# mmorise/World

Measured on AMD Instinct MI355X. Metric: analysis frames/sec (Harvest+CheapTrick+D4C, 48 kHz, 5 ms hop), higher is better.
Workload: dtype f64; 1 GPU; configs[1]: 1 x (48 kHz, 10 s) utterance(s) per step, Harvest+CheapTrick+D4C, fft_size=2048, frame_period=5 ms, inputs/outputs in HBM, 12 independent jobs in flight (one HIP stream + context each, a different utterance per job); utterances_per_gpu=1, jobs_in_flight=12, parallelism=single GPU, no collective

## Files before the change

include/world_hip.h:

```cpp
#ifndef WORLD_HIP_H_
#define WORLD_HIP_H_

#ifdef __cplusplus
extern "C" {
#endif

#if defined(__GNUC__)
#define WORLD_HIP_API __attribute__((visibility("default")))
#else
#define WORLD_HIP_API
#endif


typedef struct {
  double f0_floor;
  double f0_ceil;
  double channels_in_octave;
  double frame_period;
  int speed;
  double allowed_range;
} DioOption;

typedef struct {
  double f0_floor;
// ... 183 lines not shown
WORLD_HIP_API int world_hip_cheaptrick_batch(WorldHipContext *ctx, int n_utt, int fs, const double *d_x,
                                             int x_stride, const int *x_length, const int *n_frames,
                                             int f_stride, const double *d_tpos, const double *d_f0,
                                             const CheapTrickOption *option, double *d_spectrogram);
WORLD_HIP_API int world_hip_d4c_batch(WorldHipContext *ctx, int n_utt, int fs, const double *d_x,
                                      int x_stride, const int *x_length, const int *n_frames,
                                      int f_stride, const double *d_tpos, const double *d_f0,
                                      int fft_size, const D4COption *option, double *d_aperiodicity);

WORLD_HIP_API int world_hip_synthesis_batch(WorldHipContext *ctx, int n_utt, int fs, double frame_period,
                                            int fft_size, const int *n_frames, int f_stride, const double *d_f0,
                                            const double *d_spectrogram, const double *d_aperiodicity,
                                            const int *y_length, int y_stride, double *d_y);

WORLD_HIP_API int world_hip_synthesis_records(WorldHipContext *ctx, int n_utt, int fs, double frame_period, int fft_size,
                                              const int *n_frames, long long first_row, const double *d_block, int cols,
                                              int wire, int number_of_dimensions, const int *y_length, int y_stride,
                                              double *d_y);

WORLD_HIP_API int world_hip_probe_machine(WorldHipContext *ctx, double *values, int n_values);
WORLD_HIP_API int world_hip_probe_rfft(WorldHipContext *ctx, int lg_n, int max_lr, int threads, int static_plan,
                                       long long batch, const double *d_in, double *d_spectrum);
WORLD_HIP_API int world_hip_probe_irfft(WorldHipContext *ctx, int lg_n, int max_lr, int threads, int static_plan,
                                        long long batch, const double *d_spectrum, double *d_out);
WORLD_HIP_API int world_hip_probe_fft(WorldHipContext *ctx, int mode, int lg_n, int max_lr, int threads, int swizzle,
                                      long long batch, const void *d_in, void *d_out);
WORLD_HIP_API int world_hip_probe_select(WorldHipContext *ctx, int mode, int threads, int K, long long rows,
                                         const double *d_keys, double *d_out);
WORLD_HIP_API int world_hip_probe_harvest_contour(WorldHipContext *ctx, int n_utt, const int *nfb, const int *nc, int maxc,
                                                  int fb_stride, const double *d_cand, const double *d_score, double frame_period,
                                                  int f_stride, double *d_pruned_cand, double *d_pruned_score, double *d_step2,
                                                  double *d_step3, double *d_step4, int sec_cap, int *d_sec_n, int *d_sec,
                                                  double *d_basic_f0, double *d_tpos, double *d_f0);

WORLD_HIP_API int world_hip_analyze_batch(WorldHipContext *ctx, int n_utt, int fs, const double *d_x, int x_stride,
                                          const int *x_length, const HarvestOption *harvest_option,
                                          const CheapTrickOption *cheaptrick_option, const D4COption *d4c_option,
                                          int f_stride, double *d_tpos, double *d_f0, double *d_spectrogram,
                                          double *d_aperiodicity);
WORLD_HIP_API int world_hip_record_columns(int fft_size, int wire);
WORLD_HIP_API int world_hip_analyze_packed(WorldHipContext *ctx, int n_utt, int fs, const double *d_x, int x_stride,
                                           const int *x_length, const HarvestOption *harvest_option,
                                           const CheapTrickOption *cheaptrick_option, const D4COption *d4c_option,
                                           long long first_row, double *d_block, int cols);
WORLD_HIP_API int world_hip_coded_columns(int fs, int number_of_dimensions);
WORLD_HIP_API int world_hip_analyze_coded(WorldHipContext *ctx, int n_utt, int fs, const double *d_x, int x_stride,
                                          const int *x_length, const HarvestOption *harvest_option,
                                          const CheapTrickOption *cheaptrick_option, const D4COption *d4c_option,
                                          int number_of_dimensions, long long first_row, double *d_block, int cols);
WORLD_HIP_API int world_hip_spectral_packed_range(WorldHipContext *ctx, int n_utt, int fs, const double *d_x, int x_stride,
                                                  const int *x_length, const int *n_frames, int f_stride,
                                                  const double *d_tpos, const double *d_f0,
                                                  const CheapTrickOption *cheaptrick_option, const D4COption *d4c_option,
                                                  int frame_lo, int frame_hi, int reuse_offsets, long long first_row,
                                                  double *d_block, int cols);
WORLD_HIP_API int world_hip_cheaptrick_batch_range(WorldHipContext *ctx, int n_utt, int fs, const double *d_x, int x_stride,
                                                   const int *x_length, const int *n_frames, int f_stride,
                                                   const double *d_tpos, const double *d_f0, const CheapTrickOption *option,
                                                   int frame_lo, int frame_hi, int reuse_offsets, double *d_spectrogram);
WORLD_HIP_API int world_hip_d4c_batch_range(WorldHipContext *ctx, int n_utt, int fs, const double *d_x, int x_stride,
                                            const int *x_length, const int *n_frames, int f_stride, const double *d_tpos,
                                            const double *d_f0, int fft_size, const D4COption *option, int frame_lo,
                                            int frame_hi, int reuse_offsets, double *d_aperiodicity);
WORLD_HIP_API int world_hip_pack_results(WorldHipContext *ctx, int n_utt, const int *n_frames, int f_stride,
                                         int bins, const double *d_tpos, const double *d_f0,
                                         const double *d_spectrogram, const double *d_aperiodicity,
// ... 186 lines not shown
```

world_amd/api.py:

```python
import ctypes as C
import os
import weakref

import numpy as np

HERE = os.path.dirname(os.path.abspath(__file__))
LIB_PATH = os.environ.get("WORLD_HIP_LIB") or os.path.join(HERE, "libworld_hip.so")

_dp = C.POINTER(C.c_double)
_ip = C.POINTER(C.c_int)


class DioOption(C.Structure):
    _fields_ = [("f0_floor", C.c_double), ("f0_ceil", C.c_double), ("channels_in_octave", C.c_double),
                ("frame_period", C.c_double), ("speed", C.c_int), ("allowed_range", C.c_double)]


class HarvestOption(C.Structure):
    _fields_ = [("f0_floor", C.c_double), ("f0_ceil", C.c_double), ("frame_period", C.c_double)]


class CheapTrickOption(C.Structure):
    _fields_ = [("q1", C.c_double), ("f0_floor", C.c_double), ("fft_size", C.c_int)]

# ... 213 lines not shown
    lib.world_hip_create.restype = vp
    lib.world_hip_create.argtypes = [C.c_int, vp]
    lib.world_hip_destroy.argtypes = [vp]
    lib.world_hip_last_error.restype = C.c_char_p
    lib.world_hip_sync.argtypes = [vp]
    lib.world_hip_workspace_bytes.restype = C.c_ulonglong
    lib.world_hip_workspace_bytes.argtypes = [vp]
    lib.world_hip_noise_table_bytes.restype = C.c_ulonglong
    lib.world_hip_noise_table_bytes.argtypes = [vp]
    lib.world_hip_verify_tables.argtypes = [vp]
    lib.world_hip_harvest_batch.argtypes = [vp, C.c_int, C.c_int, vp, C.c_int, _ip, C.POINTER(HarvestOption),
                                            C.c_int, vp, vp]
    lib.world_hip_dio_batch.argtypes = [vp, C.c_int, C.c_int, vp, C.c_int, _ip, C.POINTER(DioOption),
                                        C.c_int, vp, vp]
    lib.world_hip_stonemask_batch.argtypes = [vp, C.c_int, C.c_int, vp, C.c_int, _ip, _ip, C.c_int, vp, vp, vp]
    lib.world_hip_cheaptrick_batch.argtypes = [vp, C.c_int, C.c_int, vp, C.c_int, _ip, _ip, C.c_int, vp, vp,
                                               C.POINTER(CheapTrickOption), vp]
    lib.world_hip_d4c_batch.argtypes = [vp, C.c_int, C.c_int, vp, C.c_int, _ip, _ip, C.c_int, vp, vp, C.c_int,
                                        C.POINTER(D4COption), vp]
    lib.world_hip_synthesis_batch.argtypes = [vp, C.c_int, C.c_int, C.c_double, C.c_int, _ip, C.c_int, vp, vp, vp,
                                              _ip, C.c_int, vp]
    lib.world_hip_pcm16_to_double.argtypes = [vp, C.c_longlong, vp, vp]
    lib.world_hip_set_synthesis_pulse_capacity.argtypes = [vp, C.c_int]
    lib.world_hip_synthesis_pulses_dropped.argtypes = [vp, _ip]
    lib.world_hip_probe_rfft.argtypes = [vp, C.c_int, C.c_int, C.c_int, C.c_int, C.c_longlong, vp, vp]
    lib.world_hip_probe_irfft.argtypes = [vp, C.c_int, C.c_int, C.c_int, C.c_int, C.c_longlong, vp, vp]
    if hasattr(lib, "world_hip_probe_fft"):
        lib.world_hip_probe_fft.argtypes = [vp, C.c_int, C.c_int, C.c_int, C.c_int, C.c_int, C.c_longlong, vp, vp]
    if hasattr(lib, "world_hip_probe_select"):
        lib.world_hip_probe_select.argtypes = [vp, C.c_int, C.c_int, C.c_int, C.c_longlong, vp, vp]
    if hasattr(lib, "world_hip_probe_harvest_contour"):
        lib.world_hip_probe_harvest_contour.argtypes = [vp, C.c_int, _ip, _ip, C.c_int, C.c_int, vp, vp, C.c_double, C.c_int,
                                                        vp, vp, vp, vp, vp, C.c_int, vp, vp, vp, vp, vp]
    lib.world_hip_analyze_packed.argtypes = [vp, C.c_int, C.c_int, vp, C.c_int, _ip, C.POINTER(HarvestOption),
                                             C.POINTER(CheapTrickOption), C.POINTER(D4COption), C.c_longlong, vp, C.c_int]
    lib.world_hip_analyze_sharded.argtypes = [C.c_int, C.POINTER(vp), C.c_int, C.c_int, C.POINTER(vp), _ip,
                                              C.POINTER(HarvestOption), C.POINTER(CheapTrickOption), C.POINTER(D4COption),
                                              C.c_int, C.POINTER(vp), C.c_longlong, C.c_int, C.POINTER(C.c_longlong)]
    lib.world_hip_check_shape.argtypes = [C.c_int, C.c_int, C.c_char_p, C.c_int]
    if hasattr(lib, "world_hip_set_hint"):
        lib.world_hip_set_hint.argtypes = [vp, C.c_int]
    if hasattr(lib, "world_hip_probe_machine"):
        lib.world_hip_probe_machine.argtypes = [vp, C.POINTER(C.c_double), C.c_int]
    lib.world_hip_record_columns.argtypes = [C.c_int, C.c_int]
    if hasattr(lib, "world_hip_analyze_coded"):
        lib.world_hip_coded_columns.argtypes = [C.c_int, C.c_int]
        lib.world_hip_analyze_coded.argtypes = [vp, C.c_int, C.c_int, vp, C.c_int, _ip, C.POINTER(HarvestOption),
                                                C.POINTER(CheapTrickOption), C.POINTER(D4COption), C.c_int, C.c_longlong, vp, C.c_int]
    lib.world_hip_spectral_packed_range.argtypes = [vp, C.c_int, C.c_int, vp, C.c_int, _ip, _ip, C.c_int, vp, vp,
                                                    C.POINTER(CheapTrickOption), C.POINTER(D4COption), C.c_int, C.c_int,
                                                    C.c_int, C.c_longlong, vp, C.c_int]
    lib.world_hip_cheaptrick_batch_range.argtypes = [vp, C.c_int, C.c_int, vp, C.c_int, _ip, _ip, C.c_int, vp, vp,
                                                     C.POINTER(CheapTrickOption), C.c_int, C.c_int, C.c_int, vp]
    lib.world_hip_d4c_batch_range.argtypes = [vp, C.c_int, C.c_int, vp, C.c_int, _ip, _ip, C.c_int, vp, vp, C.c_int,
                                              C.POINTER(D4COption), C.c_int, C.c_int, C.c_int, vp]
    lib.world_hip_analyze_batch.argtypes = [vp, C.c_int, C.c_int, vp, C.c_int, _ip, C.POINTER(HarvestOption),
                                            C.POINTER(CheapTrickOption), C.POINTER(D4COption), C.c_int, vp, vp, vp, vp]
    lib.world_hip_graph_begin.argtypes = [vp]
    lib.world_hip_graph_end.argtypes = [vp, C.POINTER(vp)]
    lib.world_hip_graph_launch.argtypes = [vp, vp]
    lib.world_hip_graph_destroy.argtypes = [vp]
    lib.world_hip_pack_results.argtypes = [vp, C.c_int, _ip, C.c_int, C.c_int, vp, vp, vp, vp, C.c_longlong, vp]
    lib.world_hip_unpack_results.argtypes = [vp, C.c_int, _ip, C.c_int, C.c_int, vp, C.c_longlong, vp, vp, vp, vp]
    lib.world_hip_allgather_blocks.argtypes = [C.c_int, C.POINTER(vp), C.POINTER(vp), C.POINTER(C.c_longlong), C.c_int,
                                               C.POINTER(vp)]
    lib.world_hip_pcm_to_double.argtypes = [vp, C.c_longlong, C.c_int, vp, vp]
# ... 1014 lines not shown
                                                 out.data_ptr()), "probe_fft")
        return out

    def probe_select(self, keys, K, mode=0):
        t = self.torch
        assert keys.dtype == t.float64 and keys.is_contiguous() and keys.dim() == 3 and keys.shape[2] == 10
        out = t.empty((keys.shape[0], 3), dtype=t.float64, device=keys.device)
        self._check(self.lib.world_hip_probe_select(self._context(), mode, keys.shape[1], K, keys.shape[0], keys.data_ptr(),
                                                    out.data_ptr()), "probe_select")
        return out

    def probe_harvest_contour(self, cand, score, nfb, nc, frame_period=5.0):
        t = self.torch
        assert cand.dtype == score.dtype == t.float64 and cand.is_contiguous() and score.is_contiguous()
        assert cand.dim() == 3 and cand.shape == score.shape and len(nfb) == len(nc) == cand.shape[0]
        n, stride, maxc = cand.shape
        nfb, nc = [int(v) for v in nfb], [int(v) for v in nc]
        frames = [int((f - 1) / frame_period) + 1 for f in nfb]
        sec_cap, f_stride = max(nfb) // 2 + 4, max(max(frames), 1)
        nan = lambda *shape: t.full(shape, float("nan"), dtype=t.float64, device=cand.device)
        out = dict(pruned_cand=nan(n, stride, maxc), pruned_score=nan(n, stride, maxc), step2=nan(n, stride), step3=nan(n, stride),
                   step4=nan(n, stride), sec_n=t.full((n, 2), -1, dtype=t.int32, device=cand.device),
                   sec=t.full((n, 6, sec_cap), -1, dtype=t.int32, device=cand.device), basic_f0=nan(n, stride),
                   tpos=nan(n, f_stride), f0=nan(n, f_stride))
        ints = lambda v: (C.c_int * n)(*v)
        self._check(self.lib.world_hip_probe_harvest_contour(
            self._context(), n, ints(nfb), ints(nc), maxc, stride, cand.data_ptr(), score.data_ptr(), frame_period, f_stride,
            out["pruned_cand"].data_ptr(), out["pruned_score"].data_ptr(), out["step2"].data_ptr(), out["step3"].data_ptr(),
            out["step4"].data_ptr(), sec_cap, out["sec_n"].data_ptr(), out["sec"].data_ptr(), out["basic_f0"].data_ptr(),
            out["tpos"].data_ptr(), out["f0"].data_ptr()), "probe_harvest_contour")
        out["n_frames"] = frames
        return out

    def capture(self, fn):
        ctx = self._context()
        self._check(self.lib.world_hip_graph_begin(ctx), "graph_begin")
        g = C.c_void_p()
        try:
            fn()
        except BaseException:
            if self.lib.world_hip_graph_end(ctx, C.byref(g)) == 0 and g:
                self.lib.world_hip_graph_destroy(g)
            raise
        self._check(self.lib.world_hip_graph_end(ctx, C.byref(g)), "graph_end")
        return Graph(self, ctx, g)

    def analyze_packed(self, x, fs, block, first_row=0, x_len=None, frame_period=5.0, f0_floor=71.0, f0_ceil=800.0,
                       q1=-0.15, threshold=0.85, fft_size=None):
        t = self.torch
        B, L, xl = self._prep(x, x_len)
        fft_size = fft_size or cheaptrick_fft_size(fs, 71.0)
        nb = fft_size // 2 + 1
        nf = [frame_count(fs, int(n), frame_period) for n in xl]
        cols = block.shape[-1]
        assert block.dtype == t.float64 and block.is_contiguous() and cols in (2 + 2 * nb, 2 + nb) and block.device == x.device
        assert first_row >= 0 and first_row + sum(nf) <= block.shape[0]
        hopt, copt, dopt = HarvestOption(f0_floor, f0_ceil, frame_period), CheapTrickOption(q1, 71.0, fft_size), D4COption(threshold)
        self._check(self.lib.world_hip_analyze_packed(self._context(), B, fs, x.data_ptr(), L, xl.ctypes.data_as(_ip),
                                                      C.byref(hopt), C.byref(copt), C.byref(dopt), first_row,
                                                      block.data_ptr(), cols), "analyze_packed")
        return nf

    def analyze_coded(self, x, fs, block, first_row=0, x_len=None, frame_period=5.0, f0_floor=71.0, f0_ceil=800.0,
                      q1=-0.15, threshold=0.85, number_of_dimensions=60, fft_size=None):
        t = self.torch
        B, L, xl = self._prep(x, x_len)
# ... 627 lines not shown
```

world_amd/csrc/api.hip:

```cpp
#include "../../include/world_hip.h"

#include <algorithm>
#include <climits>
#include <cmath>
#include <cstdint>
#include <cstring>
#include <cstdarg>
#include <deque>
#include <mutex>
#include <thread>
#include <unordered_map>
#include <stdexcept>
#include <string>
#include <vector>

#include "common.h"
#include "bandfilter.h"
#include "codec.h"
#include "decimate.h"
#include "dio.h"
#include "exchange.h"
#include "fft_probe.h"
#include "d4c_select_probe.h"
#include "gmm_host.h"
// ... 427 lines not shown
  p.park_ws = slot ? a.take<double>(slot * p.park_slots) : nullptr;
}
static void spectral_workspace(WorldHipContext *c, CtParams *ct, D4cParams *d4c, const int *x_length, const int *n_frames) {
  ensure_arena(c, d4c ? measure([&](Arena &a) { carve_d4c(a, *d4c); }) : measure([&](Arena &a) { carve_cheaptrick(a, *ct); }));
  const BatchView &b = ct ? ct->b : d4c->b;
  WorldHipContext::PrepToken t;
  t.n_utt = b.n_utt; t.fs = b.fs; t.f_stride = b.f_stride; t.x_stride = b.x_stride; t.x = b.x;
  t.lengths_hash = lengths_hash(x_length, n_frames, b.n_utt);
  if (ct) {
    c->arena.reset();
    carve_cheaptrick(c->arena, *ct);
    t.fft = 1 << ct->lg_fft; t.f0 = ct->f0; t.tpos = ct->tpos; t.opt = ct->f0_floor;
    t.lo = 0; t.hi = c->arena.used;
    claim_prepared(c, c->prep_ct, c->prep_d4c, t, ct->skip_prepare != 0, "CheapTrick");
    if (!ct->skip_prepare) devrt::dpoison(c->arena.base + c->arena.floor, c->arena.used - c->arena.floor, c->stream);
  }
  if (d4c) {
    c->arena.reset();
    carve_d4c(c->arena, *d4c);
    t.fft = d4c->fft_out; t.f0 = d4c->f0; t.tpos = d4c->tpos; t.opt = d4c->threshold;
    t.lo = reinterpret_cast<char *>(d4c->ap0) - c->arena.base; t.hi = c->arena.used;
    claim_prepared(c, c->prep_d4c, c->prep_ct, t, d4c->skip_prepare != 0, "D4C");
    char *lo = reinterpret_cast<char *>(d4c->skip_prepare ? d4c->coarse : d4c->ap0);
    devrt::dpoison(lo, c->arena.base + c->arena.used - lo, c->stream);
  }
}

static std::string shape_limit(int what, int fs, int fft_size);
static void refuse_shape_limit(int what, int fs, int fft_size) {
  const std::string lim = shape_limit(what, fs, fft_size);
  if (!lim.empty()) fail("%s", lim.c_str());
}
static bool inkernel_consts() { return getenv("WORLD_HIP_INKERNEL_CONSTS") != nullptr; }
static CtParams setup_cheaptrick(WorldHipContext *c, int n_utt, int fs, const double *d_x, int x_stride,
                                 const int *x_length, const int *n_frames, int f_stride, const double *d_tpos,
                                 const double *d_f0, const CheapTrickOption *opt, double *d_sp, const RowLayout &lay,
                                 int *max_frames_out) {
  check_batch(n_utt, fs, d_x, x_stride, x_length);
  const int lg = ilog2_exact(opt->fft_size);
  const std::string lim = shape_limit(2, fs, opt->fft_size);
  if (!lim.empty()) fail("%s", lim.c_str());
  const int max_frames = *max_frames_out = max_frame_count(n_frames, n_utt, f_stride);
  CtParams p;
  p.b = batch_view(c, n_utt, fs, d_x, x_stride, x_length, n_frames, f_stride);
  p.tpos = d_tpos; p.f0 = d_f0; p.spectrogram = d_sp;
  p.out_row = lay.rows ? upload(c, std::vector<int>(lay.rows, lay.rows + n_utt)) : nullptr;
  p.out_stride = lay.stride ? lay.stride : (size_t)(opt->fft_size / 2 + 1);
  p.out_col_bytes = lay.col_bytes; p.out_f32 = lay.f32;
  p.code_ndim = lay.code_dims; p.code_knot = lay.code_knot; p.code_frac = lay.code_frac;
  p.code_w_re = lay.code_w_re; p.code_w_im = lay.code_w_im;
  if (p.code_ndim > 0 && (lay.f32 || !lay.code_knot || p.code_ndim > opt->fft_size / 4 + 1)) fail("CheapTrick: bad coded-row layout");
  p.f0_floor = 3.0 * fs / (opt->fft_size - 3.0);
  p.noise = ensure_noise(c, (size_t)max_frames * ct_max_draws_per_frame(opt->fft_size));
  p.tab = c->tab;
  p.q1 = opt->q1;
  p.lg_fft = lg;
  p.frec = nullptr;
  p.frame_consts = inkernel_consts() ? 0 : 1;
  p.frame_threads = ct_frame_threads(lg);
  p.lift0 = (1.0 - 2.0 * opt->q1) + 2.0 * opt->q1;
  if (lay.frame_lo < 0 || lay.frame_hi < lay.frame_lo) fail("bad frame range [%d, %d)", lay.frame_lo, lay.frame_hi);
  p.frame_lo = lay.frame_lo; p.frame_hi = lay.frame_hi; p.skip_prepare = lay.skip_prepare ? 1 : 0;
  return p;
}
static void run_cheaptrick(WorldHipContext *c, int n_utt, int fs, const double *d_x, int x_stride,
                           const int *x_length, const int *n_frames, int f_stride, const double *d_tpos,
// ... 261 lines not shown
  static const int ev_group_env = [] { const char *e = getenv("WORLD_HIP_EVENT_GROUP"); return e ? std::max(1, atoi(e)) : 40; }();
  p.ev_group = std::min(n_utt, ev_group_env);
  p.ev_u0 = 0;
  const size_t E = p.ev_group;
  p.nyq_slices = (max_y + 4095) / 4096;
  p.mean_parts = p.ratio == 1 ? p.nyq_slices : (max_x + 2 * p.lag + 2 * kDecPad + kDecSpan - 1) / kDecSpan;
  begin_stage(c, [&](Arena &a) {
    p.nyq = a.take<double>(B * p.nyq_slices * 4);
    p.mean_part = a.take<double>(B * p.mean_parts);
    p.quirk = a.take<double>(B * p.nch * kQuirkDoubles);
    p.fwd = a.take<double>(B * p.m_stride);
    p.y = a.take<double>(B * p.y_stride);
    p.events = a.take<double>(E * p.nch * 4 * p.ev_cap);
    p.ev_count = a.take<int>(E * p.nch * 4);
    if (direct_lists) {
      p.seg_events = p.events; p.seg_count = p.ev_count;
    } else {
      p.seg_events = a.take<double>(E * p.nch * 4 * p.nseg * p.seg_cap);
      p.seg_count = a.take<int>(E * p.nch * 4 * p.nseg);
    }
    p.blk_spec = a.take<double2>(B * p.nblk * kBandFftBins);
    p.raw = a.take<double>(B * p.nch * p.fb_stride);
    carve_harvest_tail(a, p, B);
  });
  p.b = batch_view(c, n_utt, fs, d_x, x_stride, x_length, nfr.data(), f_stride);
  p.y_len = upload(c, yl);
  p.nfb = upload(c, nfb);
  p.ref_fft = upload(c, rfft);
  p.band_f0 = hb.d_band_f0; p.band_half = hb.d_half; p.band_off = hb.d_off; p.band_taps = hb.d_taps;
  p.win_tab = hb.d_win_tab; p.win_lane = hb.d_win_tab + (size_t)hb.win_tab_len * 6;
  p.win_full = hb.win_full_entries && !getenv("WORLD_HIP_REFINE_ROTATE")
                   ? reinterpret_cast<const double2 *>(p.win_lane + (size_t)hb.win_tab_len * WAVE * 2) : nullptr;
  p.refine_frames = getenv("WORLD_HIP_REFINE_FRAMES") != nullptr;
  p.inkernel_consts = inkernel_consts() ? 1 : 0;
  p.tpos = d_tpos; p.f0 = d_f0;
  launch_harvest(p, max_x, max_y, max_fb, max_fr, c->stream);
#ifdef WORLD_EMU
  if (const char *dump = getenv("WORLD_EMU_DUMP")) {
    auto put = [&](const char *tag, const void *ptr, size_t bytes) {
      std::string fn = std::string(dump) + "_" + tag + ".bin";
      FILE *f = fopen(fn.c_str(), "wb"); fwrite(ptr, 1, bytes, f); fclose(f);
    };
    int hdr[6] = {p.nch, p.fb_stride, p.maxc, max_fb, p.y_stride, yl[0]};
    put("hdr", hdr, sizeof hdr);
    put("y", p.y, sizeof(double) * p.y_stride);
    put("raw", p.raw, sizeof(double) * p.nch * p.fb_stride);
    put("cand_a", p.cand_a, sizeof(double) * p.fb_stride * p.maxc);
    put("cand_b", p.cand_b, sizeof(double) * p.fb_stride * p.maxc);
    put("score_a", p.score_a, sizeof(double) * p.fb_stride * p.maxc);
    put("score_b", p.score_b, sizeof(double) * p.fb_stride * p.maxc);
    put("basic", p.basic_f0, sizeof(double) * p.fb_stride);
    put("nc", p.nc, sizeof(int));
  }
#endif
}

static void prepare_dio_bands(WorldHipContext *c, int fs, const DioOption *opt, int ratio) {
  DioBands &db = c->dio_bands;
  if (db.fs == fs && db.ratio == ratio && db.f0_floor == opt->f0_floor && db.f0_ceil == opt->f0_ceil &&
      db.cpo == opt->channels_in_octave && db.nb > 0)
    return;
  const double afs = static_cast<double>(fs) / ratio;
  const int nb = 1 + static_cast<int>(log(opt->f0_ceil / opt->f0_floor) / kLog2 * opt->channels_in_octave);
  std::vector<double> fb(nb), taps, lowcut;
  std::vector<int> hal(nb), off(nb);
  int max_ntap = 0;
// ... 1903 lines not shown
    const size_t B = n_utt, row = p.fb_stride, cand_bytes = sizeof(double) * B * row * maxc;
    refuse_overlap(me,
                   {{d_pruned_cand, cand_bytes, "pruned_cand"}, {d_pruned_score, cand_bytes, "pruned_score"},
                    {d_step2, sizeof(double) * B * row, "step2"}, {d_step3, sizeof(double) * B * row, "step3"},
                    {d_step4, sizeof(double) * B * row, "step4"}, {d_basic_f0, sizeof(double) * B * row, "basic_f0"},
                    {d_sec_n, sizeof(int) * B * 2, "sec_n"}, {d_sec, sizeof(int) * B * 6 * p.sec_cap, "sec"},
                    {d_tpos, sizeof(double) * B * f_stride, "tpos"}, {d_f0, sizeof(double) * B * f_stride, "f0"}},
                   {{d_cand, cand_bytes, "cand"}, {d_score, cand_bytes, "score"}});
    begin_stage(c, [&](Arena &a) { carve_harvest_tail(a, p, B); });
    p.b.n_utt = n_utt; p.b.f_stride = f_stride;
    p.b.n_frames = upload(c, nfr);
    p.nfb = upload(c, fb);
    devrt::d2d(p.nc, upload(c, cn), sizeof(int) * B, c->stream);
    for (size_t u = 0; u < B; ++u) {
      const size_t at = u * row * maxc, n = sizeof(double) * fb[u] * maxc;
      devrt::d2d(p.cand_b + at, d_cand + at, n, c->stream);
      devrt::d2d(p.score_b + at, d_score + at, n, c->stream);
    }
    p.tpos = d_tpos; p.f0 = d_f0;
    launch_harvest_tail(p, max_fb, max_fr, c->stream);
    for (size_t u = 0; u < B; ++u) {
      const size_t at = u * row * maxc, n = sizeof(double) * fb[u] * maxc, f = u * row, nf = sizeof(double) * fb[u];
      if (cn[u]) {
        devrt::d2d(d_pruned_cand + at, p.cand_a + at, n, c->stream);
        devrt::d2d(d_pruned_score + at, p.score_a + at, n, c->stream);
      }
      devrt::d2d(d_step2 + f, p.c2 + f, nf, c->stream);
      devrt::d2d(d_step3 + f, p.c3 + f, nf, c->stream);
      devrt::d2d(d_step4 + f, p.c0 + f, nf, c->stream);
      devrt::d2d(d_basic_f0 + f, p.basic_f0 + f, nf, c->stream);
    }
    devrt::d2d(d_sec_n, p.sec_n, sizeof(int) * B * 2, c->stream);
    devrt::d2d(d_sec, p.sec, sizeof(int) * B * 6 * p.sec_cap, c->stream);
  });
}

int world_hip_pack_results(WorldHipContext *c, int n_utt, const int *n_frames, int f_stride, int bins,
                           const double *d_tpos, const double *d_f0, const double *d_spectrogram,
                           const double *d_aperiodicity, long long first_row, double *d_block) {
  return guarded(c, [&] {
    run_pack(c, false, n_utt, n_frames, f_stride, bins, d_tpos, d_f0, d_spectrogram, d_aperiodicity, first_row, d_block);
  });
}

int world_hip_unpack_results(WorldHipContext *c, int n_utt, const int *n_frames, int f_stride, int bins,
                             const double *d_block, long long first_row, double *d_tpos, double *d_f0,
                             double *d_spectrogram, double *d_aperiodicity) {
  return guarded(c, [&] {
    run_pack(c, true, n_utt, n_frames, f_stride, bins, d_tpos, d_f0, d_spectrogram, d_aperiodicity, first_row,
             const_cast<double *>(d_block));
  });
}

int world_hip_allgather_blocks(int n_dev, WorldHipContext *const *ctxs, const double *const *d_src, const long long *rows,
                               int cols, double *const *d_dst) {
  try {
    if (n_dev <= 0 || !ctxs || !d_src || !rows || !d_dst || cols <= 0) fail("bad arguments");
    std::vector<long long> first(n_dev + 1, 0);
    for (int d = 0; d < n_dev; ++d) {
      if (!ctxs[d] || rows[d] < 0 || (rows[d] > 0 && !d_src[d]) || !d_dst[d]) fail("bad block %d", d);
      for (int e = 0; e < d; ++e)
        if (ctxs[e] == ctxs[d]) fail("context %d listed twice", d);
      first[d + 1] = first[d] + rows[d];
    }
    std::vector<std::unique_lock<std::mutex>> locks;
    {
// ... 460 lines not shown
```

world_amd/csrc/bandfilter.h:

```cpp
#pragma once
#include "trace.h"
#include "common.h"

namespace world_hip {

constexpr int kBpThreads = 256;
constexpr int kOutPer = 8;
constexpr int kTile = kBpThreads * kOutPer;
constexpr int kSegTiles = 2;
constexpr int kSeg = kTile * kSegTiles;
constexpr int kSegCap = kSeg / 2 + 2;

__host__ __device__ __forceinline__ int pad8(int i) { return i + (i >> 3); }

struct BandJob {
  const double *in;
  int in_len;
  int n;
  const double *taps;
  int ntap;
  int shift;
  int max_ntap;
  int nseg;
  double *seg_events;
// ... 347 lines not shown
    base = base < lo + 1 ? lo + 1 : base;
    base = base > hi - 32 ? hi - 32 : base;
    const int ones = ones_at(base + sub, true);
    if (ones == 0) hi = base;
    else if (ones == 32) lo = base + 31;
    else return base + ones;
  }
  while (hi - lo > 32) {
    const int stride = (hi - lo + 31) / 32;
    const int idx = lo + (sub + 1) * stride;
    const int ones = ones_at(idx, idx < hi);
    const int nlo = lo + ones * stride, nhi = lo + (ones + 1) * stride;
    lo = nlo;
    hi = nhi < hi ? nhi : hi;
  }
  return lo + 1 + ones_at(lo + 1 + sub, lo + 1 + sub < hi);
#endif
}

__device__ __forceinline__ double interp_intervals(const double *e, int n_int, double fs, double t) {
  const int lo = intervals_at_or_before(e, n_int, fs, t);
  int k = lo < 1 ? 1 : (lo > n_int - 1 ? n_int - 1 : lo);
  double x0 = interval_loc(e, k - 1, fs), x1 = interval_loc(e, k, fs);
  double y0 = interval_f0(e, k - 1, fs), y1 = interval_f0(e, k, fs);
  double sl = (t - x0) / (x1 - x0);
  return y0 + sl * (y1 - y0);
}

struct IntervalRange {
  int c_first, c_last;
  int j_lo, m;
};
#ifndef HV_INTERVAL_CAP
#define HV_INTERVAL_CAP 288
#endif
constexpr int kIntervalCap = HV_INTERVAL_CAP;

__device__ __forceinline__ void interval_range_ends(const double *e, int n_int, double fs, double t, bool last,
                                                    IntervalRange *r) {
  const int c = intervals_at_or_before(e, n_int, fs, t);
  if (last) r->c_last = c; else r->c_first = c;
}
__device__ __forceinline__ void interval_range_close(int n_int, IntervalRange *r) {
  const int k_first = r->c_first < 1 ? 1 : (r->c_first > n_int - 1 ? n_int - 1 : r->c_first);
  const int k_last = r->c_last < 1 ? 1 : (r->c_last > n_int - 1 ? n_int - 1 : r->c_last);
  r->j_lo = k_first - 1;
  r->m = k_last - r->j_lo + 1;
}
__device__ __forceinline__ double interp_staged(const IntervalRange &r, const double *loc, const double *f0,
                                                int n_int, double t) {
  int lo = r.c_first, hi = r.c_last;
  while (lo < hi) {
    const int mid = (lo + hi) >> 1;
    if (loc[mid - r.j_lo] <= t) lo = mid + 1; else hi = mid;
  }
  const int k = (lo < 1 ? 1 : (lo > n_int - 1 ? n_int - 1 : lo)) - r.j_lo;
  const double x0 = loc[k - 1], x1 = loc[k], y0 = f0[k - 1], y1 = f0[k];
  const double sl = (t - x0) / (x1 - x0);
  return y0 + sl * (y1 - y0);
}

}
```

world_amd/csrc/harvest.h:

```cpp
#pragma once
#include "common.h"

namespace world_hip {

constexpr int kQuirkDoubles = 8;
constexpr int kBandFftThreads = 256;
struct HarvestParams {
  BatchView b;
  double f0_floor, f0_ceil, frame_period;
  int ratio;
  double afs;
  int nch;
  int maxc;
  int lag;
  int y_stride;
  int fb_stride;
  int ev_cap;
  int refine_cap;
  int sec_cap;
  int lone_job;
  int ext_cap;
  const int *y_len;
  const int *nfb;
  const double *band_f0;
  const int *band_half;
  const int *band_off;
  const double *band_taps;
  const double2 *band_spec;
  double2 *blk_spec;
  int fft_seg;
  int fft_pre;
  int max_half;
  const int *ref_fft;
  double *nyq;
  int nyq_slices;
  double *mean_part;
  int mean_parts;
  double *quirk;
  int inkernel_consts;
  const double *win_tab;
  const double *win_lane;
  const double2 *win_full;
  int refine_frames;
  Tables tab;
  double *fwd;
  int m_stride;
  double *y;
  double *seg_events;
  int *seg_count;
  int nseg;
  int seg_cap;
  int nblk;
  int chunk_blocks;
  double *events;
  int *ev_count;
  int ev_group;
  int ev_u0;
  double *raw;
  double *cand_a, *score_a;
  double *cand_b, *score_b;
  int *nc;
  double *c0, *c2, *c3;
  int *sec;
  int *sec_n;
  double *sec_sum;
  double *ext;
  double *basic_f0;
  double *tpos;
  double *f0;
};

inline int hv_sliced_sections(int max_fb) { return max_fb / 7 + 4; }
inline int hv_section_rows(int max_fb) { return max_fb / 2 + 4; }
constexpr int kBandFftLg = 12, kBandFft = 1 << kBandFftLg, kBandFftBins = kBandFft / 2 + 1;
int hv_fft_segment(int max_half);
void launch_band_spectra(const double *d_taps, const int *d_off, const int *d_half, int nch, double2 *d_spec,
                         const Tables &tab, hipStream_t stream);
void launch_harvest(const HarvestParams &p, int max_x_len, int max_y_len, int max_fb, int max_frames,
                    hipStream_t stream);
void launch_harvest_tail(const HarvestParams &p, int max_fb, int max_frames, hipStream_t stream);
void launch_harvest_contour(const HarvestParams &p, int max_fb, int max_frames, hipStream_t stream);

}
```

world_amd/csrc/harvest.hip:

```cpp
#ifndef HV_PLAIN_TID
#define WH_FRESH_TID
#endif
#include "bandfilter.h"
#include "decimate.h"
#include "harvest.h"
#include "trace.h"
WH_TRACE_DEFINE(hv)

namespace world_hip {

__global__ void __launch_bounds__(kDecThreads) hv_decimate_fwd(HarvestParams p, IirCoef c) {
  DYN_LDS(lds);
  const int u = blockIdx.y;
  dec_forward_block(p.b.x + (size_t)u * p.b.x_stride, p.b.x_len[u], p.lag, c, blockIdx.x,
                    p.fwd + (size_t)u * p.m_stride, reinterpret_cast<double *>(lds), dec_warm(p.ratio));
}
__global__ void __launch_bounds__(kDecThreads) hv_decimate_bwd(HarvestParams p, IirCoef c) {
  DYN_LDS(lds);
  const int u = blockIdx.y;
  dec_backward_block(p.fwd + (size_t)u * p.m_stride, p.b.x_len[u], p.lag, p.ratio, c, blockIdx.x,
                     p.lag / p.ratio, p.y_len[u], p.y + (size_t)u * p.y_stride, reinterpret_cast<double *>(lds),
                     dec_warm(p.ratio), p.mean_part + (size_t)u * p.mean_parts);
}
__global__ void hv_copy_signal(HarvestParams p) {
// ... 256 lines not shown
#endif
constexpr int kRawRun = HV_RAW_RUN;
__device__ __forceinline__ double hv_gate(const HarvestParams &p, int band, double v0, double v1, double v2, double v3) {
  double c = (v0 + v1 + v2 + v3) / 4.0;
  const double fb = p.band_f0[band];
  if (c > fb * 1.1 || c < fb * 0.9 || c > p.f0_ceil || c < p.f0_floor) c = 0.0;
  return c;
}
#ifndef HV_RAW_MIN_WG
#define HV_RAW_MIN_WG 8
#endif
__global__ void __launch_bounds__(kRawFrames, HV_RAW_MIN_WG) hv_raw_candidates(HarvestParams p) {
  DYN_LDS(lds);
  const int band = blockIdx.x, ue = blockIdx.z, u = ue + p.ev_u0, tid = threadIdx.x, nt = blockDim.x;
  if (band >= p.nch) return;
  const int f_begin = blockIdx.y * kRawRun, f_end = imin(f_begin + kRawRun, p.nfb[u]);
  if (f_begin >= f_end) return;
  const int *cnt = p.ev_count + (ue * p.nch + band) * 4;
  const double *ev = p.events + ((size_t)(ue * p.nch + band) * 4) * p.ev_cap;
  double *out = p.raw + ((size_t)u * p.nch + band) * p.fb_stride;
  int n_int[4];
  bool ok = true;
  for (int fam = 0; fam < 4; ++fam) {
    n_int[fam] = cnt[fam] >= 2 ? cnt[fam] - 1 : 0;
    if (n_int[fam] - 2 <= 0) ok = false;
  }
  if (!ok) {
    for (int f = f_begin + tid; f < f_end; f += nt) out[f] = 0.0;
    return;
  }
  double *loc = reinterpret_cast<double *>(lds);
  double *fz = loc + 4 * kIntervalCap;
  IntervalRange *range = reinterpret_cast<IntervalRange *>(fz + 4 * kIntervalCap);
#ifdef WORLD_EMU
  for (int job = tid; job < 8; job += nt) {
    const int fam = job >> 1;
    const bool last = job & 1;
    interval_range_ends(ev + (size_t)fam * p.ev_cap, n_int[fam], p.afs, (last ? f_end - 1 : f_begin) * 1 / 1000.0, last,
                        range + fam);
  }
#else
  {
    static_assert(kRawFrames == 8 * 32, "one 32-lane group per (family, end)");
    const int job = tid >> 5, fam = job >> 1, sub = tid & 31;
    const bool last = job & 1;
    const int c = intervals_at_or_before_group(ev + (size_t)fam * p.ev_cap, n_int[fam], p.afs,
                                               (last ? f_end - 1 : f_begin) * 1 / 1000.0, (tid >> 5) & 1, sub);
    if (sub == 0) { if (last) range[fam].c_last = c; else range[fam].c_first = c; }
  }
#endif
  __syncthreads();
  for (int fam = tid; fam < 4; fam += nt) interval_range_close(n_int[fam], range + fam);
  __syncthreads();
  const bool staged = range[0].m <= kIntervalCap && range[1].m <= kIntervalCap && range[2].m <= kIntervalCap &&
                      range[3].m <= kIntervalCap;
  if (!staged) {
    for (int f = f_begin + tid; f < f_end; f += nt) {
      const double t = f * 1 / 1000.0;
      out[f] = hv_gate(p, band, interp_intervals(ev, n_int[0], p.afs, t), interp_intervals(ev + p.ev_cap, n_int[1], p.afs, t),
                       interp_intervals(ev + 2 * (size_t)p.ev_cap, n_int[2], p.afs, t),
                       interp_intervals(ev + 3 * (size_t)p.ev_cap, n_int[3], p.afs, t));
    }
    return;
  }
  {
    const int m0 = range[0].m, m1 = m0 + range[1].m, m2 = m1 + range[2].m, m3 = m2 + range[3].m;
    for (int job = tid; job < m3; job += nt) {
      const int fam = (job >= m0) + (job >= m1) + (job >= m2);
      const int i = job - (fam == 0 ? 0 : fam == 1 ? m0 : fam == 2 ? m1 : m2);
      const double *e = ev + (size_t)fam * p.ev_cap + range[fam].j_lo;
      loc[fam * kIntervalCap + i] = interval_loc(e, i, p.afs);
      fz[fam * kIntervalCap + i] = interval_f0(e, i, p.afs);
    }
  }
  __syncthreads();
  for (int f = f_begin + tid; f < f_end; f += nt) {
    const double t = f * 1 / 1000.0;
    double v[4];
#pragma unroll
    for (int fam = 0; fam < 4; ++fam)
      v[fam] = interp_staged(range[fam], loc + fam * kIntervalCap, fz + fam * kIntervalCap, n_int[fam], t);
    out[f] = hv_gate(p, band, v[0], v[1], v[2], v[3]);
  }
}

__global__ void hv_detect(HarvestParams p) {
  const int frame = flat_thread_x(), u = blockIdx.y;
  if (frame >= p.nfb[u]) return;
  const double *raw = p.raw + (size_t)u * p.nch * p.fb_stride + frame;
  double *out = p.cand_a + ((size_t)u * p.fb_stride + frame) * p.maxc;
  int cnt = 0, st = 0, prev = 0;
  double run_sum = 0.0;
  constexpr int kBatch = 19;
  auto fetch = [&](double (&v)[kBatch], int j0) __attribute__((always_inline)) {
#pragma unroll
    for (int q = 0; q < kBatch; ++q) v[q] = raw[(size_t)imin(j0 + q, p.nch - 1) * p.fb_stride];
  };
  auto walk = [&](const double (&v)[kBatch], int j0) __attribute__((always_inline)) {
#pragma unroll
    for (int q = 0; q < kBatch; ++q) {
      const int j = j0 + q;
      if (j >= p.nch || j == 0) continue;
      const int cur = (j == p.nch - 1) ? 0 : (v[q] > 0 ? 1 : 0);
      if (cur - prev == 1) { st = j; run_sum = 0.0; }
      if (cur - prev == -1 && j - st >= 10 && cnt < p.maxc) out[cnt++] = run_sum / (j - st);
      if (cur) run_sum += v[q];
      prev = cur;
    }
  };
  double va[kBatch], vb[kBatch];
  fetch(va, 0);
  for (int j0 = 0; j0 < p.nch; j0 += 2 * kBatch) {
    fetch(vb, j0 + kBatch);
    walk(va, j0);
// ... 510 lines not shown
      }
    }
  }
  __syncthreads();
  {
    const int lane = lane_id(), nfr = imin(kPruneFrames, nfb - f0);
    for (int r = wave_in_block(); r < nfr; r += waves_per_block()) {
      const double *c = rows + (size_t)(r + 1) * nslot, *sv = kept_sc + (size_t)r * nslot;
      double best = 0.0, top = 0.0;
      int slot = 0x7FFFFFFF;
      for (int j = lane; j < nslot; j += WAVE) {
        const double sj = sv[j];
        if (sj > top) { best = c[j]; top = sj; slot = j; }
      }
      const double wtop = wave_max(top);
      double v = 0.0;
      if (wtop > 0.0) {
        const int mine = top == wtop ? slot : 0x7FFFFFFF;
        const int win = -wave_max_int(-mine);
#ifndef WORLD_EMU
        v = readlane_f64(best, __builtin_amdgcn_readfirstlane(win % WAVE));
#else
        (void)win;
        v = best;
#endif
      }
      if (lane == 0) p.c0[(size_t)u * p.fb_stride + f0 + r] = v;
    }
  }
}

size_t hv_band_lds_bytes(int max_half) { return band_lds_bytes(2 * max_half + 1); }

void launch_harvest(const HarvestParams &p, int max_x_len, int max_y_len, int max_fb, int max_frames,
                    hipStream_t stream) {
  const int B = p.b.n_utt;
  if (p.ratio == 1) {
    WH_THREADS(hv_copy_signal, max_y_len, B, 1, stream, p);
  } else {
    IirCoef c = decimate_coef(p.ratio);
    const int spans = (max_x_len + 2 * p.lag + 2 * kDecPad + kDecSpan - 1) / kDecSpan;
    WH_BLOCKS(hv_decimate_fwd, dim3(spans, B), kDecThreads, dec_lds_bytes(), stream, p, c);
    WH_BLOCKS(hv_decimate_bwd, dim3(spans, B), kDecThreads, dec_lds_bytes(), stream, p, c);
  }
  if (p.ratio == 1) WH_BLOCKS(hv_partial_sums, dim3(p.mean_parts, B), 256, 64 * sizeof(double), stream, p);
  WH_BLOCKS(hv_remove_mean, dim3(p.nyq_slices, B), 256, 64 * sizeof(double), stream, p);
  const size_t lds = sizeof(double) * (kBandFft + 64 + twiddle_lds_doubles(kBandFftLg - 1));
  if (p.fft_seg > 0) WH_BLOCKS(hv_block_spectra, dim3(p.nblk + p.nch, B), 256, lds, stream, p);
  else WH_BLOCKS(hv_band_quirk, dim3(p.nch, B), 64, 64 * sizeof(double), stream, p);
  for (int u0 = 0; u0 < B; u0 += p.ev_group) {
    HarvestParams g = p;
    g.ev_u0 = u0;
    const int G = imin(p.ev_group, B - u0);
    if (p.fft_seg > 0 && p.inkernel_consts)
      devrt::launch_blocks("hv_band_events_fft", hv_band_events_fft<false>, dim3(p.nch, p.nseg, G), kBandFftThreads, lds, stream, g);
    else if (p.fft_seg > 0)
      devrt::launch_blocks("hv_band_events_fft", hv_band_events_fft<true>, dim3(p.nch, p.nseg, G), kBandFftThreads, lds, stream, g);
    else WH_BLOCKS(hv_band_events, dim3(p.nseg, p.nch, G), kBpThreads, hv_band_lds_bytes(p.max_half), stream, g);
    if (!(p.fft_seg > 0 && p.nseg == 1)) WH_BLOCKS(hv_compact_events, dim3(p.nch * 4, G), 256, compact_lds_bytes(p.nseg), stream, g);
    WH_BLOCKS(hv_raw_candidates, dim3((p.nch + 7) / 8 * 8, (max_fb + kRawRun - 1) / kRawRun, G), kRawFrames,
              8 * kIntervalCap * sizeof(double) + 4 * sizeof(IntervalRange), stream, g);
  }
  WH_THREADS(hv_detect, max_fb, B, 1, stream, p);
  if (p.win_full && !p.refine_frames)
    WH_WAVES(hv_refine, max_fb, B, 1, sizeof(double) * (3 * p.refine_cap + 6 * static_cast<int>(p.afs / 1000.0) + 2), stream, p);
  else
    WH_WAVES(hv_refine_frames, max_fb, B, 1, 3 * sizeof(double) * p.refine_cap, stream, p);
  launch_harvest_tail(p, max_fb, max_frames, stream);
}

void launch_harvest_tail(const HarvestParams &p, int max_fb, int max_frames, hipStream_t stream) {
  const int B = p.b.n_utt;
  WH_BLOCKS(hv_prune, dim3((max_fb + kPruneFrames - 1) / kPruneFrames, B), 256,
            sizeof(double) * (size_t)(2 * kPruneFrames + 2) * p.maxc, stream, p);
  launch_harvest_contour(p, max_fb, max_frames, stream);
}

}
```

Baseline: 4.441 million frames/s.

## Locate interpolation intervals in Harvest raw candidates by histogram scan instead of bisection

The raw-candidate kernel now histograms, per frame, how many event intervals start before it, using packed 16-bit LDS atomics, then runs a block-wide prefix scan so each frame reads its bracketing interval directly instead of bisecting per family. An optional early gate, enabled by an environment variable, writes zero for frames whose interpolated candidates provably fall outside the band's gate range. The interval cap shrinks slightly to make room for the extra LDS, and a probe entry point is added for testing the routes. The trade is per-block atomics, a scan, and more LDS against the removed binary searches; the counting path is the default.

```diff
diff --git a/include/world_hip.h b/include/world_hip.h
--- a/include/world_hip.h
+++ b/include/world_hip.h
@@ -239,6 +239,9 @@
                                                   int f_stride, double *d_pruned_cand, double *d_pruned_score, double *d_step2,
                                                   double *d_step3, double *d_step4, int sec_cap, int *d_sec_n, int *d_sec,
                                                   double *d_basic_f0, double *d_tpos, double *d_f0);
+WORLD_HIP_API int world_hip_probe_raw_candidates(WorldHipContext *ctx, int route, int n_band, int ev_cap, const double *d_events,
+                                                 const int *ev_count, const double *d_band_f0, int nfb, double afs,
+                                                 double f0_floor, double f0_ceil, int fb_stride, double *d_raw);
 
 WORLD_HIP_API int world_hip_analyze_batch(WorldHipContext *ctx, int n_utt, int fs, const double *d_x, int x_stride,
                                           const int *x_length, const HarvestOption *harvest_option,
diff --git a/world_amd/api.py b/world_amd/api.py
--- a/world_amd/api.py
+++ b/world_amd/api.py
@@ -269,6 +269,9 @@
     if hasattr(lib, "world_hip_probe_harvest_contour"):
         lib.world_hip_probe_harvest_contour.argtypes = [vp, C.c_int, _ip, _ip, C.c_int, C.c_int, vp, vp, C.c_double, C.c_int,
                                                         vp, vp, vp, vp, vp, C.c_int, vp, vp, vp, vp, vp]
+    if hasattr(lib, "world_hip_probe_raw_candidates"):
+        lib.world_hip_probe_raw_candidates.argtypes = [vp, C.c_int, C.c_int, C.c_int, vp, _ip, vp, C.c_int, C.c_double, C.c_double,
+                                                       C.c_double, C.c_int, vp]
     lib.world_hip_analyze_packed.argtypes = [vp, C.c_int, C.c_int, vp, C.c_int, _ip, C.POINTER(HarvestOption),
                                              C.POINTER(CheapTrickOption), C.POINTER(D4COption), C.c_longlong, vp, C.c_int]
     lib.world_hip_analyze_sharded.argtypes = [C.c_int, C.POINTER(vp), C.c_int, C.c_int, C.POINTER(vp), _ip,
@@ -1349,6 +1352,19 @@
         out["n_frames"] = frames
         return out
 
+    def probe_raw_candidates(self, events, counts, band_f0, nfb, afs=8000.0, f0_floor=71.0, f0_ceil=800.0, route=1):
+        t = self.torch
+        assert events.dtype == band_f0.dtype == t.float64 and events.is_contiguous() and band_f0.is_contiguous()
+        assert events.dim() == 3 and events.shape[1] == 4 and band_f0.shape == (events.shape[0],)
+        n, _, ev_cap = events.shape
+        flat = [int(v) for row in counts for v in row]
+        assert len(flat) == 4 * n
+        raw = t.full((n, int(nfb)), float("nan"), dtype=t.float64, device=events.device)
+        self._check(self.lib.world_hip_probe_raw_candidates(
+            self._context(), route, n, ev_cap, events.data_ptr(), (C.c_int * len(flat))(*flat), band_f0.data_ptr(), int(nfb), afs,
+            f0_floor, f0_ceil, int(nfb), raw.data_ptr()), "probe_raw_candidates")
+        return raw
+
     def capture(self, fn):
         ctx = self._context()
         self._check(self.lib.world_hip_graph_begin(ctx), "graph_begin")
diff --git a/world_amd/csrc/api.hip b/world_amd/csrc/api.hip
--- a/world_amd/csrc/api.hip
+++ b/world_amd/csrc/api.hip
@@ -483,6 +483,8 @@
   if (!lim.empty()) fail("%s", lim.c_str());
 }
 static bool inkernel_consts() { return getenv("WORLD_HIP_INKERNEL_CONSTS") != nullptr; }
+static bool raw_bisect() { return getenv("WORLD_HIP_RAW_BISECT") != nullptr; }
+static bool raw_early_gate() { return getenv("WORLD_HIP_RAW_EARLY_GATE") != nullptr; }
 static CtParams setup_cheaptrick(WorldHipContext *c, int n_utt, int fs, const double *d_x, int x_stride,
                                  const int *x_length, const int *n_frames, int f_stride, const double *d_tpos,
                                  const double *d_f0, const CheapTrickOption *opt, double *d_sp, const RowLayout &lay,
@@ -810,6 +812,8 @@
   p.win_full = hb.win_full_entries && !getenv("WORLD_HIP_REFINE_ROTATE")
                    ? reinterpret_cast<const double2 *>(p.win_lane + (size_t)hb.win_tab_len * WAVE * 2) : nullptr;
   p.refine_frames = getenv("WORLD_HIP_REFINE_FRAMES") != nullptr;
+  p.raw_bisect = raw_bisect() ? 1 : 0;
+  p.raw_early_gate = raw_early_gate() ? 1 : 0;
   p.inkernel_consts = inkernel_consts() ? 1 : 0;
   p.tpos = d_tpos; p.f0 = d_f0;
   launch_harvest(p, max_x, max_y, max_fb, max_fr, c->stream);
@@ -2779,6 +2783,41 @@
     }
     devrt::d2d(d_sec_n, p.sec_n, sizeof(int) * B * 2, c->stream);
     devrt::d2d(d_sec, p.sec, sizeof(int) * B * 6 * p.sec_cap, c->stream);
+  });
+}
+
+int world_hip_probe_raw_candidates(WorldHipContext *c, int route, int n_band, int ev_cap, const double *d_events, const int *ev_count,
+                                   const double *d_band_f0, int nfb, double afs, double f0_floor, double f0_ceil, int fb_stride,
+                                   double *d_raw) {
+  return guarded(c, [&] {
+    const char *const me = "probe_raw_candidates";
+    if (route < 0 || route > 3)
+      fail("%s: route = %d unsupported (0: as the environment says, 1: counted, 2: bisected, 3: counted with the early gate)", me, route);
+    if (n_band < 1 || n_band > 4096) fail("%s: n_band = %d outside 1 .. 4096", me, n_band);
+    if (ev_cap < 2 || ev_cap > (1 << 24)) fail("%s: ev_cap = %d outside 2 .. 2^24", me, ev_cap);
+    if (nfb < 1 || nfb > (1 << 24)) fail("%s: nfb = %d outside 1 .. 2^24", me, nfb);
+    if (fb_stride < nfb) fail("%s: fb_stride = %d is less than nfb = %d", me, fb_stride, nfb);
+    if (!(afs > 0)) fail("%s: afs must be positive", me);
+    if (!d_events || !ev_count || !d_band_f0 || !d_raw)
+      fail("%s: null buffer (%s)", me, !d_events ? "events" : !ev_count ? "ev_count" : !d_band_f0 ? "band_f0" : "raw");
+    std::vector<int> cnt(ev_count, ev_count + (size_t)n_band * 4);
+    for (size_t i = 0; i < cnt.size(); ++i)
+      if (cnt[i] < 0 || cnt[i] > ev_cap)
+        fail("%s: ev_count[%d][%d] = %d outside 0 .. ev_cap = %d", me, (int)(i / 4), (int)(i % 4), cnt[i], ev_cap);
+    refuse_overlap(me, {{d_raw, sizeof(double) * n_band * fb_stride, "raw"}},
+                   {{d_events, sizeof(double) * n_band * 4 * ev_cap, "events"}, {d_band_f0, sizeof(double) * n_band, "band_f0"}});
+    open_uploads(c);
+    HarvestParams p{};
+    p.nch = n_band; p.ev_cap = ev_cap; p.afs = afs; p.f0_floor = f0_floor; p.f0_ceil = f0_ceil; p.fb_stride = fb_stride;
+    p.events = const_cast<double *>(d_events);
+    p.ev_count = const_cast<int *>(upload(c, cnt));
+    p.ev_group = 1; p.ev_u0 = 0;
+    p.band_f0 = d_band_f0;
+    p.nfb = upload(c, &nfb, 1);
+    p.raw = d_raw;
+    p.raw_bisect = route == 0 ? (raw_bisect() ? 1 : 0) : route == 2;
+    p.raw_early_gate = route == 0 ? (raw_early_gate() ? 1 : 0) : route == 3;
+    launch_raw_candidates(p, nfb, 1, c->stream);
   });
 }
 
diff --git a/world_amd/csrc/bandfilter.h b/world_amd/csrc/bandfilter.h
--- a/world_amd/csrc/bandfilter.h
+++ b/world_amd/csrc/bandfilter.h
@@ -403,9 +403,10 @@
   int j_lo, m;
 };
 #ifndef HV_INTERVAL_CAP
-#define HV_INTERVAL_CAP 288
+#define HV_INTERVAL_CAP 272
 #endif
 constexpr int kIntervalCap = HV_INTERVAL_CAP;
+static_assert(kIntervalCap < 65536, "a run's counts are scanned in 16-bit fields");
 
 __device__ __forceinline__ void interval_range_ends(const double *e, int n_int, double fs, double t, bool last,
                                                     IntervalRange *r) {
@@ -431,4 +432,29 @@
   return y0 + sl * (y1 - y0);
 }
 
-}
+__device__ __forceinline__ int first_frame_at_or_after(double x, int f_lo, int f_hi) {
+  const double p = x * 1000.0, g = ceil(p);
+  if (g >= f_lo && g <= f_hi && p <= g * (1.0 - 0x1p-48) && p >= (g - 1.0) * (1.0 + 0x1p-48)) return static_cast<int>(g);
+  int f = !(g > f_lo) ? f_lo : (g > f_hi ? f_hi : static_cast<int>(g));
+  while (f > f_lo && x <= (f - 1) * 1 / 1000.0) --f;
+  while (f < f_hi && !(x <= f * 1 / 1000.0)) ++f;
+  return f;
+}
+
+__device__ __forceinline__ void count_interval_at(unsigned *hist, int slot, int fam) {
+  atomicAdd(hist + 2 * slot + (fam >> 1), 1u << (16 * (fam & 1)));
+}
+
+__device__ __forceinline__ bool surely_gated(const double (&y0)[4], const double (&y1)[4], double lo, double hi) {
+  double sm = 0.0, sM = 0.0, least = y0[0];
+#pragma unroll
+  for (int fam = 0; fam < 4; ++fam) {
+    const double m = y0[fam] < y1[fam] ? y0[fam] : y1[fam], M = y0[fam] < y1[fam] ? y1[fam] : y0[fam];
+    sm += m; sM += M;
+    least = m < least ? m : least;
+  }
+  if (!(least > 0.0) || !(sm > 0.0) || !(sM < __builtin_inf())) return false;
+  return sM < 4.0 * lo * (1.0 - 0x1p-40) || (sm > 4.0 * hi * (1.0 + 0x1p-40) && sM <= 2.0 * sm);
+}
+
+}
diff --git a/world_amd/csrc/harvest.h b/world_amd/csrc/harvest.h
--- a/world_amd/csrc/harvest.h
+++ b/world_amd/csrc/harvest.h
@@ -41,6 +41,8 @@
   const double *win_tab;
   const double *win_lane;
   const double2 *win_full;
+  int raw_bisect;
+  int raw_early_gate;
   int refine_frames;
   Tables tab;
   double *fwd;
@@ -78,6 +80,7 @@
                          const Tables &tab, hipStream_t stream);
 void launch_harvest(const HarvestParams &p, int max_x_len, int max_y_len, int max_fb, int max_frames,
                     hipStream_t stream);
+void launch_raw_candidates(const HarvestParams &p, int max_fb, int G, hipStream_t stream);
 void launch_harvest_tail(const HarvestParams &p, int max_fb, int max_frames, hipStream_t stream);
 void launch_harvest_contour(const HarvestParams &p, int max_fb, int max_frames, hipStream_t stream);
 
diff --git a/world_amd/csrc/harvest.hip b/world_amd/csrc/harvest.hip
--- a/world_amd/csrc/harvest.hip
+++ b/world_amd/csrc/harvest.hip
@@ -312,6 +312,11 @@
   double *loc = reinterpret_cast<double *>(lds);
   double *fz = loc + 4 * kIntervalCap;
   IntervalRange *range = reinterpret_cast<IntervalRange *>(fz + 4 * kIntervalCap);
+  unsigned *hist = reinterpret_cast<unsigned *>(range + 4);
+  double *scan_scratch = reinterpret_cast<double *>(hist + 2 * kRawRun);
+  const bool counted = !p.raw_bisect;
+  if (counted)
+    for (int i = tid; i < 2 * kRawRun; i += nt) hist[i] = 0u;
 #ifdef WORLD_EMU
   for (int job = tid; job < 8; job += nt) {
     const int fam = job >> 1;
@@ -349,17 +354,60 @@
       const int fam = (job >= m0) + (job >= m1) + (job >= m2);
       const int i = job - (fam == 0 ? 0 : fam == 1 ? m0 : fam == 2 ? m1 : m2);
       const double *e = ev + (size_t)fam * p.ev_cap + range[fam].j_lo;
-      loc[fam * kIntervalCap + i] = interval_loc(e, i, p.afs);
+      const double x = interval_loc(e, i, p.afs);
+      loc[fam * kIntervalCap + i] = x;
       fz[fam * kIntervalCap + i] = interval_f0(e, i, p.afs);
+      const int j = range[fam].j_lo + i;
+      if (counted && j >= range[fam].c_first && j < range[fam].c_last)
+        count_interval_at(hist, first_frame_at_or_after(x, f_begin + 1, f_end - 1) - f_begin, fam);
     }
   }
   __syncthreads();
-  for (int f = f_begin + tid; f < f_end; f += nt) {
+  if (!counted) {
+    for (int f = f_begin + tid; f < f_end; f += nt) {
+      const double t = f * 1 / 1000.0;
+      double v[4];
+#pragma unroll
+      for (int fam = 0; fam < 4; ++fam)
+        v[fam] = interp_staged(range[fam], loc + fam * kIntervalCap, fz + fam * kIntervalCap, n_int[fam], t);
+      out[f] = hv_gate(p, band, v[0], v[1], v[2], v[3]);
+    }
+    return;
+  }
+  const double fb = p.band_f0[band];
+  const double gate_lo = fb * 0.9 > p.f0_floor ? fb * 0.9 : p.f0_floor, gate_hi = fb * 1.1 < p.f0_ceil ? fb * 1.1 : p.f0_ceil;
+  unsigned long long before = 0;
+  for (int base = f_begin; base < f_end; base += nt) {
+    const int f = base + tid;
+    const unsigned long long h =
+        f < f_end ? (unsigned long long)hist[2 * (f - f_begin)] | ((unsigned long long)hist[2 * (f - f_begin) + 1] << 32) : 0ull;
+    unsigned long long total;
+    const unsigned long long upto = before + block_excl_scan_u64(h, &total, scan_scratch) + h;
+    before += total;
+    if (f >= f_end) continue;
     const double t = f * 1 / 1000.0;
+    int k[4];
+    double y0[4], y1[4];
+    auto count_of = [&](int fam) { return range[fam].c_first + (int)((upto >> (16 * fam)) & 0xFFFFull); };
+#pragma unroll
+    for (int fam = 0; fam < 4; ++fam) {
+      const int c = count_of(fam);
+      k[fam] = fam * kIntervalCap + (c < 1 ? 1 : (c > n_int[fam] - 1 ? n_int[fam] - 1 : c)) - range[fam].j_lo;
+      y0[fam] = fz[k[fam] - 1]; y1[fam] = fz[k[fam]];
+    }
+    if (p.raw_early_gate) {
+      bool interior = true;
+#pragma unroll
+      for (int fam = 0; fam < 4; ++fam) interior = interior && count_of(fam) >= 1 && count_of(fam) <= n_int[fam] - 1;
+      if (interior && surely_gated(y0, y1, gate_lo, gate_hi)) { out[f] = 0.0; continue; }
+    }
     double v[4];
 #pragma unroll
-    for (int fam = 0; fam < 4; ++fam)
-      v[fam] = interp_staged(range[fam], loc + fam * kIntervalCap, fz + fam * kIntervalCap, n_int[fam], t);
+    for (int fam = 0; fam < 4; ++fam) {
+      const double x0 = loc[k[fam] - 1], x1 = loc[k[fam]];
+      const double sl = (t - x0) / (x1 - x0);
+      v[fam] = y0[fam] + sl * (y1[fam] - y0[fam]);
+    }
     out[f] = hv_gate(p, band, v[0], v[1], v[2], v[3]);
   }
 }
@@ -936,6 +984,12 @@
 
 size_t hv_band_lds_bytes(int max_half) { return band_lds_bytes(2 * max_half + 1); }
 
+void launch_raw_candidates(const HarvestParams &p, int max_fb, int G, hipStream_t stream) {
+  WH_BLOCKS(hv_raw_candidates, dim3((p.nch + 7) / 8 * 8, (max_fb + kRawRun - 1) / kRawRun, G), kRawFrames,
+            8 * kIntervalCap * sizeof(double) + 4 * sizeof(IntervalRange) + 2 * kRawRun * sizeof(unsigned) +
+                kRawFrames / 64 * sizeof(double), stream, p);
+}
+
 void launch_harvest(const HarvestParams &p, int max_x_len, int max_y_len, int max_fb, int max_frames,
                     hipStream_t stream) {
   const int B = p.b.n_utt;
@@ -962,8 +1016,7 @@
       devrt::launch_blocks("hv_band_events_fft", hv_band_events_fft<true>, dim3(p.nch, p.nseg, G), kBandFftThreads, lds, stream, g);
     else WH_BLOCKS(hv_band_events, dim3(p.nseg, p.nch, G), kBpThreads, hv_band_lds_bytes(p.max_half), stream, g);
     if (!(p.fft_seg > 0 && p.nseg == 1)) WH_BLOCKS(hv_compact_events, dim3(p.nch * 4, G), 256, compact_lds_bytes(p.nseg), stream, g);
-    WH_BLOCKS(hv_raw_candidates, dim3((p.nch + 7) / 8 * 8, (max_fb + kRawRun - 1) / kRawRun, G), kRawFrames,
-              8 * kIntervalCap * sizeof(double) + 4 * sizeof(IntervalRange), stream, g);
+    launch_raw_candidates(g, max_fb, G, stream);
   }
   WH_THREADS(hv_detect, max_fb, B, 1, stream, p);
   if (p.win_full && !p.refine_frames)
```

After: 4.500 million frames/s (median of 6 runs). Within noise of the previous version (+1.3%).
